# Changfei-Fu/RUMI-SLAM

Hardware: AMD Instinct MI355X
Metric: frames/sec ORB extract+match (higher is better)
Workload: dtype u8; 1 GPU; ORB extract (640x480, 8-level pyramid, 1000 features/frame) + brute-force 256-bit Hamming match of consecutive frames (BASELINE.json configs[1]+[2]); scaling=n/a (one GPU), exchange=none

## Files before the change

### rumi_slam_amd/csrc/orb_host.hip

```cpp
#include <hip/hip_runtime.h>

#include <cstdlib>

#include <algorithm>
#include <atomic>
#include <cstdio>
#include <cstring>
#include <functional>
#include <string>
#include <thread>
#include <vector>

#include "orb_device.h"
#include "orb_octree.h"
#include "rumi_common.h"

using namespace rumi;

namespace rumi {
thread_local std::string g_lastError;
void set_error(const char *fmt, const char *a, const char *b, int line) {
    char buf[512];
    snprintf(buf, sizeof buf, fmt, a, b, line);
    g_lastError = buf;
// ... 261 lines not shown
    TRY_A(dev_alloc(&h->dPyr, (size_t)h->capArena * arena));
    TRY_A(dev_alloc(&h->dBlur, (size_t)h->capArena * arena));
    TRY_A(dev_alloc(&h->dCellBuf, C * h->capCells * h->capCellCand));
    TRY_A(dev_alloc(&h->dCellCnt, C * h->capCells));
    TRY_A(dev_alloc(&h->dCand, C * h->capCand));
    TRY_A(dev_alloc(&h->dLevelStart, C * (kMaxLevels + 1)));
    TRY_A(dev_alloc(&h->dSelPacked, C * h->capSel));
    TRY_A(dev_alloc(&h->dSelMeta, C * h->capSel));
    TRY_A(dev_alloc(&h->dSelCount, C));
    TRY_A(dev_alloc(&h->dOwner, C * h->capCand));
    TRY_A(dev_alloc(&h->dSelLevel, C * h->cfg.nlevels * h->selLevelCap));
    TRY_A(dev_alloc(&h->dSelLevelCnt, C * h->cfg.nlevels));
#undef TRY_A
    h->scratchFrames = (int)scratch; h->arenaFrames = (int)arena;
    return RUMI_OK;
}

extern "C" int rumi_orb_create(const RumiOrbConfig *cfg, RumiOrb **out) {
    if (!out) return RUMI_E_INVALID;
    *out = nullptr;
    if (!cfg || cfg->nlevels < 1 || cfg->nlevels > kMaxLevels || cfg->nfeatures < 1 || cfg->max_batch < 1 ||
        cfg->max_width < 1 || cfg->max_height < 1 || !(cfg->scale_factor > 1.0f) || cfg->blur_variant < 0 || cfg->blur_variant > 1) {
        g_lastError = "invalid RumiOrbConfig";
        return RUMI_E_INVALID;
    }
    int ndev = 0;
    if (hipGetDeviceCount(&ndev) != hipSuccess || ndev == 0) {
        g_lastError = "no HIP device visible: librumi_hip has no CPU fallback";
        return RUMI_E_NO_DEVICE;
    }
    RumiOrb *h = new RumiOrb();
    h->cfg = *cfg;
    if (cfg->device >= 0) { h->device = cfg->device; }
    else if (hipGetDevice(&h->device) != hipSuccess) h->device = 0;
    if (hipSetDevice(h->device) != hipSuccess) { delete h; g_lastError = "hipSetDevice failed"; return RUMI_E_NO_DEVICE; }
    h->tab = make_tables(cfg->nfeatures, cfg->scale_factor, cfg->nlevels);
    h->hostThreads = cfg->host_threads > 0 ? cfg->host_threads
                                           : (int)std::min<unsigned>(16u, std::max(1u, std::thread::hardware_concurrency()));
    std::vector<LevelGeom> g;
    int cells, cand, cellCand;
    if (!make_geometry(h->tab, cfg->max_width, cfg->max_height, g, &h->capArena, &cells, &cand, &cellCand)) {
        delete h;
        g_lastError = "max_width x max_height too small for the FAST cell grid at some level";
        return RUMI_E_INVALID;
    }
    int coefN = 0;
    for (int l = 1; l < cfg->nlevels; l++) coefN += 3 * (g[l].w + g[l].h);
    h->capCells = cells + cells / 8 + 16;
    h->capCellCand = cellCand + cellCand / 2 + 16;
    int candSum = 0;
    for (int l = 0; l < cfg->nlevels; l++) candSum += std::min(g[l].candCap, 65535);
    h->capCand = candSum + 64;
    h->capCoef = coefN + 64 * cfg->nlevels;
    h->capRowTab = 0;
    for (int l = 1; l < cfg->nlevels; l++) h->capRowTab += g[l].h + 8;
    h->capSel = cfg->nfeatures + 4 * cfg->nlevels + 64;
    int maxN = 0;
    for (int l = 0; l < cfg->nlevels; l++) maxN = std::max(maxN, h->tab.featuresPerLevel[l]);
    h->selLevelCap = maxN + 4 * 16 + 8;
    const size_t B = (size_t)cfg->max_batch, C = (size_t)scratch_frames(cfg->max_batch);
    int rc = RUMI_OK;
#define TRY_ALLOC(x) if ((rc = (x)) != RUMI_OK) { rumi_orb_destroy(h); return rc; }
    TRY_ALLOC(dev_alloc(&h->dP, 1));
    TRY_ALLOC(dev_alloc(&h->dCoef, (size_t)h->capCoef));
    TRY_ALLOC(dev_alloc(&h->dRowTab, (size_t)std::max(h->capRowTab, 1)));
    TRY_ALLOC(dev_alloc(&h->dIn, (size_t)((cfg->max_width + 3) & ~3) * cfg->max_height));
    TRY_ALLOC(alloc_frame_arenas(h, C, B));
    TRY_ALLOC(dev_alloc(&h->dOut1, (size_t)16 + (size_t)h->capSel * 60));
    if (hipHostMalloc((void **)&h->hIn, (size_t)((cfg->max_width + 3) & ~3) * cfg->max_height, hipHostMallocDefault) != hipSuccess ||
        hipHostMalloc((void **)&h->hOut1, (size_t)16 + (size_t)h->capSel * 60, hipHostMallocDefault) != hipSuccess) {
        rumi_orb_destroy(h); g_lastError = "pinned staging"; return RUMI_E_NO_DEVICE;
    }
    TRY_ALLOC(dev_alloc(&h->dErr, 1));
    TRY_ALLOC(pin_alloc(&h->hErr, 1));
    if (hipHostGetDevicePointer((void **)&h->dhOut1, h->hOut1, 0) != hipSuccess || hipHostGetDevicePointer((void **)&h->dhErr, h->hErr, 0) != hipSuccess) {
        (void)hipGetLastError();
        h->dhOut1 = nullptr; h->dhErr = nullptr;
    }
#undef TRY_ALLOC
    for (auto &e : h->ev)
        if (hipEventCreate(&e) != hipSuccess) { rumi_orb_destroy(h); g_lastError = "hipEventCreate"; return RUMI_E_NO_DEVICE; }
    auto make_slot = [h](int p) {
        RumiOrb::Lane &L = h->slot[p];
        return hipStreamCreateWithFlags(&L.s, hipStreamNonBlocking) == hipSuccess && hipStreamCreateWithFlags(&L.bs, hipStreamNonBlocking) == hipSuccess &&
               hipEventCreateWithFlags(&L.fork, hipEventDisableTiming) == hipSuccess && hipEventCreateWithFlags(&L.join, hipEventDisableTiming) == hipSuccess &&
               hipEventCreateWithFlags(&h->slotJoin[p], hipEventDisableTiming) == hipSuccess;
    };
    bool slotsOk = true;
    for (int p = 1; p < RumiOrb::kMaxParts && slotsOk; ++p) slotsOk = make_slot(p);
    if (!slotsOk || !make_slot(0)) { rumi_orb_destroy(h); g_lastError = "slot stream"; return RUMI_E_NO_DEVICE; }
    if (hipEventCreateWithFlags(&h->evPartFork, hipEventDisableTiming) != hipSuccess ||
        hipStreamCreateWithFlags(&h->sideStream, hipStreamNonBlocking) != hipSuccess ||
        hipEventCreateWithFlags(&h->evFork, hipEventDisableTiming) != hipSuccess ||
        hipEventCreateWithFlags(&h->evJoin, hipEventDisableTiming) != hipSuccess || hipEventCreate(&h->evB0) != hipSuccess ||
        hipEventCreate(&h->evB1) != hipSuccess) { rumi_orb_destroy(h); g_lastError = "side stream"; return RUMI_E_NO_DEVICE; }
    *out = h;
    return RUMI_OK;
}

extern "C" int rumi_orb_set_profiling(RumiOrb *h, int32_t on) {
    if (!h) return RUMI_E_INVALID;
    h->profiling = on != 0;
    return RUMI_OK;
}
extern "C" int rumi_orb_set_resident_queue(RumiOrb *h, int32_t on) {
    if (!h) return RUMI_E_INVALID;
    if (h->pending) { const int rc = rumi_orb_sync(h); if (rc != RUMI_OK) return rc; }
    if (on) {
        const int slots = on == 1 ? 4 : std::min(std::max(on, 2), (int)RumiOrb::kMaxParts);
        h->residentSlots = slots;
        const int need = (slots * std::min(kResidentSub, h->cfg.max_batch) + 23) / 24 * 24;
        if (h->scratchFrames < need || h->arenaFrames < need) {
            HIP_TRY(hipSetDevice(h->device));
            HIP_TRY(hipDeviceSynchronize());
            const size_t oldS = (size_t)h->scratchFrames, oldA = (size_t)h->arenaFrames;
            int rc = alloc_frame_arenas(h, std::max(oldS, (size_t)need), std::max(oldA, (size_t)need));
            if (rc != RUMI_OK) {
                h->residentQueue = false;
                (void)alloc_frame_arenas(h, oldS, oldA);
                g_lastError = "resident queue: device arenas";
                return rc;
            }
            h->lastFrames = 0; h->tapValid = false;
        }
    }
    h->residentQueue = on != 0;
    return RUMI_OK;
}
extern "C" int rumi_orb_wait_event(RumiOrb *h, void *hip_event) {
    if (!h) return RUMI_E_INVALID;
    h->userReady = (hipEvent_t)hip_event;
    return RUMI_OK;
}
extern "C" int rumi_orb_stage_ms(RumiOrb *h, float ms[8]) {
    if (!h || !ms) return RUMI_E_INVALID;
    for (int i = 0; i < 8; i++) ms[i] = h->stageMs[i];
    return RUMI_OK;
}

extern "C" int rumi_orb_sync(RumiOrb *h) {
    if (!h) return RUMI_E_INVALID;
    if (!h->pending) return RUMI_OK;
    HIP_TRY(hipSetDevice(h->device));
    HIP_TRY(hipStreamSynchronize(h->pendingStream));
    h->pending = false;
    const int err = *h->hErr;
    if (err & 16) { g_lastError = "FAST candidate capacity exceeded (more than 65535 in one level)"; return RUMI_E_CAPACITY; }
    if (err & 1) { g_lastError = "aspect ratio gives 0 or more than 16 quadtree roots"; return RUMI_E_INVALID; }
    if (err & 2) { g_lastError = "quadtree node pool exhausted"; return RUMI_E_INVALID; }
    if (err & (4 | 8)) { g_lastError = "more key-points than the handle's selection capacity"; return RUMI_E_CAPACITY; }
    return RUMI_OK;
}

extern "C" int rumi_orb_extract_batch_device(RumiOrb *h, const void *d_imgs, int32_t nframes, int32_t w, int32_t hgt,
                                             int32_t stride, int64_t frame_stride, int32_t lap0, int32_t lap1,
                                             void *d_kp, void *d_desc, void *d_counts, int32_t cap, void *hip_stream) {
    const int rc = rumi_orb_extract_batch_device_async(h, d_imgs, nframes, w, hgt, stride, frame_stride, lap0, lap1, d_kp, d_desc, d_counts, cap, hip_stream);
    if (rc != RUMI_OK) { if (h && h->pending) (void)rumi_orb_sync(h); return rc; }
    return rumi_orb_sync(h);
}

struct OutLayout { void *kp; long long kpStride; void *desc; long long descStride; void *counts; long long countsStride; };

static int extract_async_impl(RumiOrb *h, const void *d_imgs, int32_t nframes, int32_t w, int32_t hgt, int32_t stride, int64_t frame_stride,
                              int32_t lap0, int32_t lap1, const OutLayout &out, int32_t cap, void *hip_stream) {
    void *d_kp = out.kp, *d_desc = out.desc, *d_counts = out.counts;
    if (!h || !d_imgs || !d_kp || !d_desc || !d_counts || nframes < 1 || cap < 1 || stride < w) {
        g_lastError = "rumi_orb_extract_batch_device: bad argument";
        return RUMI_E_INVALID;
    }
    if (w <= 0 || hgt <= 0) return RUMI_E_EMPTY;
    if (nframes > h->cfg.max_batch) { g_lastError = "nframes > max_batch"; return RUMI_E_CAPACITY; }
    if (h->scratchFrames <= 0 || h->arenaFrames <= 0) { g_lastError = "the handle has no device arenas (an earlier rumi_orb_set_resident_queue failed to allocate them)"; return RUMI_E_CAPACITY; }
    HIP_TRY(hipSetDevice(h->device));
    int rc;
    if (h->pending && (h->gw != w || h->gh != hgt) && (rc = rumi_orb_sync(h)) != RUMI_OK) return rc;
    rc = set_geometry(h, w, hgt);
    if (rc != RUMI_OK) return rc;
    hipStream_t st = (hipStream_t)hip_stream;
    if (h->pending && (st != h->pendingStream || h->profiling)) { rc = rumi_orb_sync(h); if (rc != RUMI_OK) return rc; }
    const DevParams &P = h->hP;
    bool stagedL0 = false;
    if ((reinterpret_cast<uintptr_t>(d_imgs) & 3) || (stride & 3) || (frame_stride & 3)) {
        stagedL0 = true;
        const int wp = (w + 3) & ~3;
        if (!h->dL0) HIP_TRY(hipMalloc((void **)&h->dL0, (size_t)((h->cfg.max_width + 3) & ~3) * h->cfg.max_height * h->cfg.max_batch));
        for (int f = 0; f < nframes; f++)
            HIP_TRY(hipMemcpy2DAsync(h->dL0 + (size_t)f * wp * hgt, wp, (const uint8_t *)d_imgs + (long long)f * frame_stride, stride, w, hgt,
                                     hipMemcpyDeviceToDevice, st));
        d_imgs = h->dL0; stride = wp; frame_stride = (int64_t)wp * hgt;
    }
    ImgSrc src{(const uint8_t *)d_imgs, frame_stride, stride, h->dPyr, h->dBlur};
    const bool prof = h->profiling;
    float acc[8] = {0};
    h->tapValid = false;

    static const bool serial = std::getenv("RUMI_SERIAL") != nullptr;
    const int parts = (!prof && !serial) ? std::min(4, std::max(nframes / 32, 1)) : 1;
    bool clearInKernel = !h->pending && parts == 1 && !(h->residentQueue && !prof && !serial && !h->feed) && P.nlevels > 1;
    if (!h->pending && !clearInKernel) HIP_TRY(hipMemsetAsync(h->dErr, 0, sizeof(int32_t), st));
    if (h->userReady && !(h->residentQueue && !prof && !serial && !h->feed)) { HIP_TRY(hipStreamWaitEvent(st, h->userReady, 0)); h->userReady = nullptr; }
    const bool resident = h->residentQueue && !prof && !serial && !h->feed;
    using Lane = RumiOrb::Lane;
    auto lane_of = [&](int slot) -> Lane {
        if (slot || resident) return h->slot[slot];
        return {st, serial || prof ? st : h->sideStream, h->evFork, h->evJoin};
    };
    const bool fuseBlur = !prof && !serial && nframes < 16 && fast_blur_fusable(P);
    const bool tilePyramid = !prof && !serial && nframes <= 4 && h->nPyrTiles > 0;
    auto stage_a = [&](const ImgSrc &ps, int n, const Lane &L) -> int {
        hipStream_t s = L.s;
        if (prof) HIP_TRY(hipEventRecord(h->ev[0], s));
        if (tilePyramid) {
            launch_pyramid_tiles(h->dP, ps, h->dCoef, h->dRowTab, h->dPyrTiles, h->nPyrTiles, h->pyrBuf, h->pyrTab, n, s, clearInKernel ? h->dErr : nullptr);
            clearInKernel = false;
        } else
        for (int l = 1; l < P.nlevels; l++) {
            launch_resize(h->dP, P, ps, h->dCoef, h->dRowTab, l, n, s, clearInKernel ? h->dErr : nullptr);
            clearInKernel = false;
        }
        if (prof) HIP_TRY(hipEventRecord(h->ev[1], s));
        if (fuseBlur) return RUMI_OK;
        HIP_TRY(hipEventRecord(L.fork, s));
        HIP_TRY(hipStreamWaitEvent(L.bs, L.fork, 0));
        if (prof) HIP_TRY(hipEventRecord(h->evB0, L.bs));
        launch_blur(h->dP, P, ps, n, h->cfg.blur_variant, L.bs);
        if (prof) HIP_TRY(hipEventRecord(h->evB1, L.bs));
        HIP_TRY(hipEventRecord(L.join, L.bs));
        HIP_TRY(hipGetLastError());
        return RUMI_OK;
    };
    if (h->hostImagePending) {
        h->hostImagePending = false;
        HIP_TRY(hipMemcpyAsync(h->dIn, h->hIn, (size_t)stride * hgt, hipMemcpyHostToDevice, st));
    }
    if (parts == 1 && !resident) {
        if (h->feed && (rc = h->feed(nframes, st)) != RUMI_OK) return rc;
        if ((rc = stage_a(src, nframes, lane_of(0))) != RUMI_OK) return rc;
    }

    auto run_part = [&](int frame0, int n, int scr0, const Lane &L, bool timed, bool withStageA, int arena0) -> int {
        hipStream_t s = L.s;
        ImgSrc ps = src;
        ps.l0 = src.l0 + (long long)frame0 * frame_stride;
        ps.pyr = src.pyr + (long long)(arena0 >= 0 ? arena0 : frame0) * P.arenaStride;
        ps.blur = src.blur + (long long)(arena0 >= 0 ? arena0 : frame0) * P.arenaStride;
        if (withStageA) { const int ra = stage_a(ps, n, L); if (ra != RUMI_OK) return ra; }
        uint32_t *cellBuf = h->dCellBuf + (size_t)scr0 * P.totalCells * P.maxCellCand;
        int32_t *cellCnt = h->dCellCnt + (size_t)scr0 * P.totalCells;
        uint32_t *candp = h->dCand + (size_t)scr0 * P.totalCand;
        int32_t *lvStart = h->dLevelStart + (size_t)scr0 * (kMaxLevels + 1);
        uint32_t *selLevel = h->dSelLevel + (size_t)scr0 * P.nlevels * h->selLevelCap;
        int32_t *selLevelCnt = h->dSelLevelCnt + (size_t)scr0 * P.nlevels;
        uint32_t *selPacked = h->dSelPacked + (size_t)scr0 * h->capSel, *selMeta = h->dSelMeta + (size_t)scr0 * h->capSel;
        if (timed) HIP_TRY(hipEventRecord(h->ev[3], s));
        if (fuseBlur) (void)launch_fast_blur(h->dP, P, ps, cellBuf, cellCnt, n, h->cfg.blur_variant, s);
        else launch_fast(h->dP, P, ps, cellBuf, cellCnt, n, s);
        if (timed) HIP_TRY(hipEventRecord(h->ev[4], s));
        launch_compact(h->dP, P, cellBuf, cellCnt, candp, lvStart, h->dErr, n, s);
        if (timed) HIP_TRY(hipEventRecord(h->ev[5], s));
        launch_octree(h->dP, P, candp, lvStart, h->dOwner + (size_t)scr0 * P.totalCand, selLevel, selLevelCnt, h->selLevelCap, h->dErr, n, h->octLds, s);
        const bool fuseAssemble = !timed && !serial && n <= 4 && (long long)((h->capSel + 7) / 8) * n <= 2048;
        int32_t *countsOut = (int32_t *)((uint8_t *)d_counts + (size_t)frame0 * out.countsStride);
        if (!fuseAssemble)
            launch_assemble(h->dP, selLevel, selLevelCnt, h->selLevelCap, lap0, lap1, selPacked, selMeta, h->dSelCount + scr0, h->capSel,
                            countsOut, out.countsStride, h->dErr, n, s, h->zeroCopyOut ? h->dhErr : nullptr);
        if (timed) HIP_TRY(hipEventRecord(h->ev[6], s));
        if (!fuseBlur) HIP_TRY(hipStreamWaitEvent(s, L.join, 0));
        if (fuseAssemble)
            launch_assemble_orient_desc(h->dP, ps, selLevel, selLevelCnt, h->selLevelCap, lap0, lap1, countsOut, out.countsStride, h->dErr,
                                        h->zeroCopyOut ? h->dhErr : nullptr, selPacked, selMeta, h->dSelCount + scr0, h->capSel, h->capSel,
                                        (RumiKeyPoint *)((uint8_t *)d_kp + (size_t)frame0 * out.kpStride), out.kpStride,
                                        (uint8_t *)d_desc + (size_t)frame0 * out.descStride, out.descStride, cap, n, s);
        else
        launch_orient_desc(h->dP, ps, selPacked, selMeta, h->dSelCount + scr0, h->capSel, h->capSel,
                           (RumiKeyPoint *)((uint8_t *)d_kp + (size_t)frame0 * out.kpStride), out.kpStride,
                           (uint8_t *)d_desc + (size_t)frame0 * out.descStride, out.descStride, cap, n, s);
        if (timed) HIP_TRY(hipEventRecord(h->ev[7], s));
        const RumiOrb::Mirror &mr = h->mirror;
        if (mr.host) HIP_TRY(hipMemcpyAsync(mr.host + (size_t)frame0 * mr.row, mr.dev + (size_t)frame0 * mr.row, (size_t)n * mr.row, hipMemcpyDeviceToHost, s));
        return RUMI_OK;
    };
    if (resident) {
        constexpr int kMaxSlots = RumiOrb::kMaxParts;
        const int kSlots = h->residentSlots;
        const int slotFrames = h->scratchFrames / kSlots;
        const int cap64 = std::min(kResidentSub, slotFrames);
        const int nsub = (nframes + cap64 - 1) / cap64, sub = (nframes + nsub - 1) / nsub;
        const bool fork = !h->pending || !h->lastResident || stagedL0;
        if (fork) HIP_TRY(hipEventRecord(h->evPartFork, st));
        bool touched[kMaxSlots] = {false, false, false, false, false, false, false, false};
        for (int j = 0, base = 0; base < nframes; j++, base += sub) {
            const int n = std::min(sub, nframes - base), slot = (h->rot + j) % kSlots;
            const Lane L = lane_of(slot);
            if (fork && !touched[slot]) HIP_TRY(hipStreamWaitEvent(L.s, h->evPartFork, 0));
            if (h->userReady && !touched[slot]) HIP_TRY(hipStreamWaitEvent(L.s, h->userReady, 0));
            touched[slot] = true;
            rc = run_part(base, n, slot * slotFrames, L, false, true, slot * slotFrames);
            if (rc != RUMI_OK) return rc;
            h->lastChunkBase = base; h->lastChunkFrames = n; h->lastChunkSlot = slot * slotFrames;
        }
        h->rot = (h->rot + nsub) % kSlots;
        h->userReady = nullptr;
        for (int p = 0; p < kSlots; p++)
            if (touched[p]) {
// ... 322 lines not shown
```

### rumi_slam_amd/csrc/orb_kernels.hip

```cpp
#include <hip/hip_runtime.h>

#include "orb_device.h"
#include "orb_math.h"

namespace rumi {

struct PatternF { float v[256 * 4]; };
constexpr PatternF make_pattern_f() {
    constexpr int8_t src[256 * 4] = {
#include "orb_pattern.inc"
    };
    PatternF p{};
    for (int i = 0; i < 256 * 4; i++) p.v[i] = (float)src[i];
    return p;
}
__constant__ PatternF c_patternF = make_pattern_f();

__device__ __forceinline__ unsigned xcd_swizzle(unsigned lin, unsigned total) {
    const unsigned q = total >> 3, r = total & 7, xcd = lin & 7;
    return (xcd < r ? xcd * (q + 1) : r * (q + 1) + (xcd - r) * q) + (lin >> 3);
}

struct __attribute__((packed)) U32 { uint32_t v; };
struct __attribute__((packed)) U64 { uint64_t v; };
// ... 499 lines not shown
    if (r0 < rps && c < g.nd) {
        const uint8_t *src = g.img + r0 * g.pitch + 4 * c;
        uint8_t *dst = tile + r0 * TP + 4 * c;
        const int nb = (g.rows + rps - 1) / rps, lastRow = g.rows - rps;
        uint32_t v[kStageDepth];
#pragma unroll
        for (int j = 0; j < kStageDepth; j++)
            if (j < nb) v[j] = reinterpret_cast<const U32 *>(src + (long long)min(j * rps, lastRow) * g.pitch)->v;
#pragma unroll
        for (int j = 0; j < kStageDepth; j++)
            if (j < nb) *reinterpret_cast<uint32_t *>(dst + min(j * rps, lastRow) * TP) = v[j];
        for (int j = kStageDepth; j < nb; j++)
            *reinterpret_cast<uint32_t *>(dst + min(j * rps, lastRow) * TP) = reinterpret_cast<const U32 *>(src + (long long)min(j * rps, lastRow) * g.pitch)->v;
    }
}

template <int TPC>
__device__ __forceinline__ void fast_cell_process(const DevParams *__restrict__ P, const FastLds &F, const FastCell &g, uint8_t *tile, uint8_t *sc,
                                                  uint32_t *__restrict__ cellBuf, int32_t *__restrict__ cellCnt, int lane) {
    const int TP = TPC ? TPC : F.tp;
    const int dw = g.cols - 6, dh = g.rows - 6;
    const unsigned Mdw = magic_of(dw), Mtp = magic_of(TP);
    for (int idx = lane * 16; idx < (dh + 2) * TP; idx += 1024) *reinterpret_cast<uint4 *>(&sc[idx]) = make_uint4(0, 0, 0, 0);
    wave_lds_fence();
    const int npx = dw * dh;
    const int scDelta = -2 * TP - 3;
    uint16_t *cl = reinterpret_cast<uint16_t *>(sc + F.scBytes);
    uint16_t *sl = cl + kRingCap;
    int thr = max(1, P->iniTh);
    uint32_t *out = cellBuf + g.cellIdx * P->maxCellCand;
    int found;
#pragma nounroll
    for (int pass = 0;; pass++) {
        const int nScored = fast_score_cell_bytes<TPC>(tile, sc, cl, sl, TP, dw, dh, thr, lane);
        wave_lds_fence();
        const bool listed = nScored <= kScoredCap;
        const int nItems = listed ? nScored : npx;
        found = 0;
        for (int base = 0; base < nItems; base += 128) {
            int si[2];
            bool in[2];
#pragma unroll
            for (int h = 0; h < 2; h++) {
                const int k = base + 64 * h + lane;
                in[h] = k < nItems;
                if (listed) {
                    si[h] = (int)sl[in[h] ? k : 0] + scDelta;
                } else {
                    const int kk = in[h] ? k : 0, py = magic_div(kk, Mdw);
                    si[h] = mul24(py + 1, TP) + (kk - mul24(py, dw)) + 1;
                }
            }
            int v[2];
            bool isMax[2];
#pragma unroll
            for (int h = 0; h < 2; h++) {
                const uint8_t *s = &sc[si[h]];
                v[h] = s[0];
                const int n0 = s[-TP - 1], n1 = s[-TP], n2 = s[-TP + 1], n3 = s[-1], n4 = s[1], n5 = s[TP - 1], n6 = s[TP], n7 = s[TP + 1];
                isMax[h] = in[h] & (v[h] > 0) & (v[h] > n0) & (v[h] > n1) & (v[h] > n2) & (v[h] > n3) & (v[h] > n4) & (v[h] > n5) & (v[h] > n6) & (v[h] > n7);
            }
            const unsigned long long b0 = __ballot(isMax[0]), b1 = __ballot(isMax[1]);
            const int c0 = __popcll(b0);
#pragma unroll
            for (int h = 0; h < 2; h++) {
                if (isMax[h]) {
                    const unsigned long long b = h ? b1 : b0;
                    const int slot = __builtin_amdgcn_mbcnt_hi((uint32_t)(b >> 32), __builtin_amdgcn_mbcnt_lo((uint32_t)b, found + (h ? c0 : 0)));
                    const int py1 = magic_div(si[h], Mtp), px1 = si[h] - mul24(py1, TP);
                    const uint32_t x = (uint32_t)(px1 + 2 + g.ox), y = (uint32_t)(py1 + 2 + g.oy);
                    out[slot] = x | (y << 12) | ((uint32_t)v[h] << 24);
                }
            }
            found += c0 + __popcll(b1);
        }
        if (found > 0 || pass == 1) break;
        thr = max(1, P->minTh);
    }
    if (lane == 0) cellCnt[g.cellIdx] = found;
}

template <int TPC>
__device__ __forceinline__ void fast_cells_body(const DevParams *__restrict__ P, const ImgSrc &src, const FastLds &F, uint32_t *__restrict__ cellBuf,
                                                int32_t *__restrict__ cellCnt, unsigned bx, unsigned gx) {
    extern __shared__ __attribute__((aligned(16))) uint8_t fl[];
    const int lane = threadIdx.x & 63, wave = __builtin_amdgcn_readfirstlane(threadIdx.x >> 6);
    const unsigned wg = xcd_swizzle(blockIdx.y * gx + bx, gx * gridDim.y);
    const int wpg = blockDim.x >> 6;
    const int cell = (wg % gx) * wpg + wave, frame = wg / gx;
    uint8_t *tile = fl + (size_t)wave * F.perWave;
    uint8_t *sc = tile + F.tileBytes;
    const int TP = TPC ? TPC : F.tp;
    const FastCell gA = fast_cell_geom(P, src, cell, frame, cellCnt, lane);
    if (!gA.live) return;
    fast_cell_stage<TPC>(gA, tile, TP, lane);
    fast_cell_process<TPC>(P, F, gA, tile, sc, cellBuf, cellCnt, lane);
}
template <int TPC>
__global__ __launch_bounds__(256) void k_fast_cells(const DevParams *__restrict__ P, ImgSrc src, FastLds F,
                                                    uint32_t *__restrict__ cellBuf, int32_t *__restrict__ cellCnt) {
    fast_cells_body<TPC>(P, src, F, cellBuf, cellCnt, blockIdx.x, gridDim.x);
}

constexpr int kCompactThreads = 256;
__global__ __launch_bounds__(kCompactThreads) void k_compact(const DevParams *__restrict__ P, const uint32_t *__restrict__ cellBuf,
                                                 const int32_t *__restrict__ cellCnt, uint32_t *__restrict__ cand,
                                                 int32_t *__restrict__ levelStart, int32_t *__restrict__ errFlag) {
    extern __shared__ int sStart[];
    __shared__ int part[kCompactThreads];
    const int tid = threadIdx.x, frame = blockIdx.x;
    const int nc = P->totalCells;
    const int32_t *cnt = cellCnt + (long long)frame * nc;
    const int chunk = (nc + kCompactThreads - 1) / kCompactThreads;
    int sum = 0;
    for (int k = 0; k < chunk; k++) {
        const int c = tid * chunk + k;
        if (c < nc) sum += cnt[c];
    }
    const int lane = tid & 63, wave = __builtin_amdgcn_readfirstlane(tid >> 6);
    int inc = sum;
#pragma unroll
    for (int o = 1; o < 64; o <<= 1) {
        const int t = __shfl_up(inc, o);
        if (lane >= o) inc += t;
    }
    if (lane == 63) part[wave] = inc;
    __syncthreads();
    int base = 0, total = 0;
#pragma unroll
    for (int w = 0; w < kCompactThreads / 64; w++) {
        const int t = part[w];
        if (w < wave) base += t;
        total += t;
    }
    if (tid == 0) sStart[nc] = total;
    int run = base + inc - sum;
    for (int k = 0; k < chunk; k++) {
        const int c = tid * chunk + k;
        if (c < nc) { sStart[c] = run; run += cnt[c]; }
    }
    __syncthreads();
    int32_t *ls = levelStart + (long long)frame * (kMaxLevels + 1);
    if (blockIdx.y == 0 && tid <= P->nlevels) {
        const int c = tid < P->nlevels ? P->lv[tid].cellBase : nc;
        ls[tid] = sStart[c];
    }
    if (blockIdx.y == 0 && tid < P->nlevels) {
        const int c0 = P->lv[tid].cellBase, c1 = c0 + P->lv[tid].nCells;
        if (sStart[c1] - sStart[c0] > P->lv[tid].candCap) atomicOr(errFlag, 16);
    }
    uint32_t *out = cand + (long long)frame * P->totalCand;
    const int nOut = min(sStart[nc], P->totalCand);
    const uint32_t *inBase = cellBuf + (long long)frame * nc * P->maxCellCand;
    for (int j = blockIdx.y * kCompactThreads + tid; j < nOut; j += kCompactThreads * gridDim.y) {
        int lo = 0, hi = nc;
        while (hi - lo > 1) {
            const int mid = (lo + hi) >> 1;
            if (sStart[mid] <= j) lo = mid; else hi = mid;
        }
        out[j] = inBase[(long long)lo * P->maxCellCand + (j - sStart[lo])];
    }
}

constexpr int kBlurRowsSmall = 16, kBlurRowsBatch = 64;

struct BlurGrid { int base[kMaxLevels + 1]; int gx[kMaxLevels]; int bw[kMaxLevels]; };
__device__ __forceinline__ uint32_t mad_u24(uint32_t a, uint32_t b, uint32_t c) {
    uint32_t r;
    asm("v_mad_u32_u24 %0, %1, %2, %3" : "=v"(r) : "v"(a), "v"(b), "v"(c));
    return r;
}
template <int VARIANT, int kBlurRows>
__device__ __forceinline__ void blur_body(const DevParams *__restrict__ P, const ImgSrc &src, const BlurGrid &G, unsigned bxg, unsigned gxg) {
    constexpr uint32_t kT2 = VARIANT ? 49u : 48u, kT3 = VARIANT ? 55u : 56u;
    const int lane = threadIdx.x & 63, wave = __builtin_amdgcn_readfirstlane(threadIdx.x >> 6);
    const unsigned wg = xcd_swizzle(blockIdx.y * gxg + bxg, gxg * gridDim.y);
    const int frame = wg / gxg, lin = wg % gxg;
    int level = 0;
    for (int l = 1; l < P->nlevels; l++)
        if (lin >= G.base[l]) level = l;
    const DevLevel &L = P->lv[level];
    const int bx = (lin - G.base[level]) % G.gx[level], by = (lin - G.base[level]) / G.gx[level];
    const int bw = G.bw[level];
    const int xa = bx * bw + lane * 4;
    const int y0 = (by * 4 + wave) * kBlurRows;
    if (y0 >= L.h) return;
    int pitch;
    const uint8_t *img = level_base(src, P, level, frame, &pitch);
    uint8_t *out = src.blur + (long long)frame * P->arenaStride + L.off;
    const int w = L.w, h = L.h;
    const int xLast = (w - 1) & ~3;
    const int xl = min(xa, xLast);
    const bool firstBlock = bx == 0;
    const bool edgeWave = bx * bw + bw + 4 > w;
    const bool produce = lane * 4 < bw && xa < w;
    uint32_t selA = 0x03020100u, selB = 0x07060504u;
    if (edgeWave && xa + 3 >= w && xa <= xLast + 4) {
#pragma unroll
        for (int i = 0; i < 4; i++) {
            const int x = xa + i;
            if (x < w) continue;
            const int sx = 2 * (w - 1) - x, d = (xa - (sx & ~3)) >> 2;
            const uint32_t a = (d == 1 ? 4u : 0u) + (uint32_t)(sx & 3);
            const uint32_t b = d == 0 ? 4u + (uint32_t)(sx & 3) : (uint32_t)i;
            selA = (selA & ~(0xFFu << (8 * i))) | (a << (8 * i));
            selB = (selB & ~(0xFFu << (8 * i))) | (b << (8 * i));
        }
    }
    int ring[7][4];
#pragma unroll
    for (int k = 0; k < 7; k++)
#pragma unroll
        for (int i = 0; i < 4; i++) ring[k][i] = 0;
    const int yEnd = min(y0 + kBlurRows, h), rEnd = yEnd + 3;
    uint8_t *orow = out + (long long)(y0 - 6) * L.pitch + xa - L.pitch;
    const int haloOff = lane == 0 ? (firstBlock ? 0 : -4) : (lane == 63 && !edgeWave && bw == 256 ? 4 : 0);
    uint32_t Cn[7], Hn[7];
    auto fetch = [&](int r, uint32_t &C, uint32_t &H) {
        const int rc = min(r, rEnd - 1);
        const int rr = rc < 0 ? -rc : (rc >= h ? 2 * (h - 1) - rc : rc);
        const uint8_t *row = img + (long long)rr * pitch + xl;
        C = *reinterpret_cast<const uint32_t *>(row);
        H = 0;
        if (haloOff) H = *reinterpret_cast<const uint32_t *>(row + haloOff);
    };
#pragma unroll
    for (int j = 0; j < 7; j++) fetch(y0 - 3 + j, Cn[j], Hn[j]);
    uint32_t Cm[7], Hm[7];
    auto walk7 = [&](const uint32_t (&Cc)[7], const uint32_t (&Hc)[7], int r0) {
#pragma unroll
        for (int j = 0; j < 7; j++) {
            const int r = r0 + j;
            if (r >= rEnd) break;
            orow += L.pitch;
            uint32_t C = Cc[j];
            if (edgeWave) {
                const uint32_t c1 = __shfl_up(C, 1), c2 = __shfl_up(c1, 1);
                C = __builtin_amdgcn_perm(C, __builtin_amdgcn_perm(c1, c2, selA), selB);
            }
            uint32_t Lw = __shfl_up(C, 1), Rw = __shfl_down(C, 1);
            if (lane == 0) Lw = firstBlock ? __builtin_amdgcn_perm(C, C, 0x01020300u) : Hc[j];
            if (lane == 63 && !edgeWave && bw == 256) Rw = Hc[j];
            constexpr uint32_t tA = 18u | (34u << 8) | (kT2 << 16) | (kT3 << 24), tB = kT2 | (34u << 8) | (18u << 16);
            const uint32_t A0 = __builtin_amdgcn_alignbyte(C, Lw, 1), A1 = __builtin_amdgcn_alignbyte(C, Lw, 2), A2 = __builtin_amdgcn_alignbyte(C, Lw, 3);
            const uint32_t B0 = __builtin_amdgcn_alignbyte(Rw, C, 1), B1 = __builtin_amdgcn_alignbyte(Rw, C, 2), B2 = __builtin_amdgcn_alignbyte(Rw, C, 3);
            ring[j][0] = (int)__builtin_amdgcn_udot4(B0, tB, __builtin_amdgcn_udot4(A0, tA, 0u, false), false);
            ring[j][1] = (int)__builtin_amdgcn_udot4(B1, tB, __builtin_amdgcn_udot4(A1, tA, 0u, false), false);
            ring[j][2] = (int)__builtin_amdgcn_udot4(B2, tB, __builtin_amdgcn_udot4(A2, tA, 0u, false), false);
            ring[j][3] = (int)__builtin_amdgcn_udot4(Rw, tB, __builtin_amdgcn_udot4(C, tA, 0u, false), false);
            const int y = r - 3;
            if (y >= y0 && produce) {
                uint32_t o[4];
#pragma unroll
                for (int i = 0; i < 4; i++) {
                    uint32_t acc = mad_u24(kT3, (uint32_t)ring[(j + 4) % 7][i], 32768u);
                    acc = mad_u24(kT2, (uint32_t)(ring[(j + 3) % 7][i] + ring[(j + 5) % 7][i]), acc);
                    acc = mad_u24(34u, (uint32_t)(ring[(j + 2) % 7][i] + ring[(j + 6) % 7][i]), acc);
                    acc = mad_u24(18u, (uint32_t)(ring[(j + 1) % 7][i] + ring[j][i]), acc);
                    if (VARIANT) acc = min(acc, 0x00FFFFFFu);
                    o[i] = acc;
                }
                const uint32_t p01 = __builtin_amdgcn_perm(o[1], o[0], 0x0c0c0602u), p23 = __builtin_amdgcn_perm(o[3], o[2], 0x06020c0cu);
                *reinterpret_cast<uint32_t *>(orow) = p01 | p23;
            }
        }
    };
    for (int r0 = y0 - 3; r0 < rEnd; r0 += 7) {
#pragma unroll
        for (int j = 0; j < 7; j++) Cm[j] = Cn[j], Hm[j] = Hn[j];
        if (r0 + 7 < rEnd) {
#pragma unroll
            for (int j = 0; j < 7; j++) fetch(r0 + 7 + j, Cn[j], Hn[j]);
        }
        walk7(Cm, Hm, r0);
    }
}
template <int VARIANT, int kBlurRows>
__global__ __launch_bounds__(256) void k_blur(const DevParams *__restrict__ P, ImgSrc src, BlurGrid G) {
    blur_body<VARIANT, kBlurRows>(P, src, G, blockIdx.x, gridDim.x);
}
template <int TPC, int VARIANT>
__global__ __launch_bounds__(256) void k_fast_blur(const DevParams *__restrict__ P, ImgSrc src, FastLds F, uint32_t *__restrict__ cellBuf,
                                                   int32_t *__restrict__ cellCnt, BlurGrid G, unsigned gxFast) {
    if (blockIdx.x < gxFast) fast_cells_body<TPC>(P, src, F, cellBuf, cellCnt, blockIdx.x, gxFast);
    else blur_body<VARIANT, kBlurRowsSmall>(P, src, G, blockIdx.x - gxFast, gridDim.x - gxFast);
}

__device__ __forceinline__ int half_wave_sum(int v) {
    v += __builtin_amdgcn_update_dpp(0, v, 0x111, 0xF, 0xF, false);
    v += __builtin_amdgcn_update_dpp(0, v, 0x112, 0xF, 0xF, false);
    v += __builtin_amdgcn_update_dpp(0, v, 0x114, 0xF, 0xF, false);
    v += __builtin_amdgcn_update_dpp(0, v, 0x118, 0xF, 0xF, false);
    v += __builtin_amdgcn_update_dpp(0, v, 0x142, 0xA, 0xF, false);
    const int lo = __builtin_amdgcn_readlane(v, 31), hi = __builtin_amdgcn_readlane(v, 63);
    return (threadIdx.x & 32) ? hi : lo;
}
__device__ __forceinline__ int wave_sum(int v) {
#pragma unroll
    for (int o = 32; o > 0; o >>= 1) v += __shfl_xor(v, o);
    return v;
}

constexpr int kDiscP = 48, kPatchP = 48;
constexpr int kKpPerWg = 8;

struct AssembleArgs {
    const uint32_t *selLevel; const int32_t *selLevelCnt; int selLevelCap, lap0, lap1;
    int32_t *counts; long long countsStride; int32_t *errFlag, *errMirror;
    uint32_t *selPackedOut, *selMetaOut; int32_t *selCountOut;
};
template <int kKpGroups, bool kAssemble>
__global__ __launch_bounds__(256, 7) void k_orient_desc(const DevParams *__restrict__ P, ImgSrc src,
                                                     const uint32_t *__restrict__ selPacked,
                                                     const uint32_t *__restrict__ selMeta,
                                                     const int32_t *__restrict__ selCount, int selCap,
                                                     RumiKeyPoint *__restrict__ kpOut, long long kpStride, uint8_t *__restrict__ descOut,
                                                     long long descStride, int outCap, AssembleArgs A) {
    static_assert(kDiscP == kPatchP, "the disc and the patch share their rows");
    __shared__ __attribute__((aligned(16))) uint8_t sWin[kKpPerWg][37 * kPatchP];
    __shared__ __attribute__((aligned(16))) float sPat[256 * 4];
    __shared__ int4 sLv[kMaxLevels];
    __shared__ float2 sLvF[kMaxLevels];
    reinterpret_cast<float4 *>(sPat)[threadIdx.x] = reinterpret_cast<const float4 *>(c_patternF.v)[threadIdx.x];
    if (threadIdx.x < (unsigned)P->nlevels) {
        const DevLevel &Lv = P->lv[threadIdx.x];
        sLv[threadIdx.x] = threadIdx.x == 0 ? make_int4(0, src.l0Pitch, (int)Lv.off, Lv.pitch) : make_int4((int)Lv.off, Lv.pitch, (int)Lv.off, Lv.pitch);
        sLvF[threadIdx.x] = make_float2(Lv.scale, Lv.patchSize);
    }
    const int lane = threadIdx.x & 31, hw = threadIdx.x >> 5;
    const unsigned wg = xcd_swizzle(blockIdx.y * gridDim.x + blockIdx.x, gridDim.x * gridDim.y);
    const int kb = (wg % gridDim.x) * (kKpPerWg * kKpGroups) + hw, frame = wg / gridDim.x;
    int cnt;
    __shared__ uint32_t sOwnPk[kAssemble ? kKpPerWg * kKpGroups : 1], sOwnMt[kAssemble ? kKpPerWg * kKpGroups : 1];
    if constexpr (!kAssemble) {
        cnt = selCount[frame];
        __syncthreads();
    } else {
        __shared__ int sLvStart[kMaxLevels + 1], sRed[2], sOwnF[kKpPerWg * kKpGroups];
        const int nl = P->nlevels, tid = threadIdx.x;
        if (tid == 0) {
            int run = 0;
            for (int l = 0; l < nl; l++) { sLvStart[l] = run; run += A.selLevelCnt[(long long)frame * nl + l]; }
            sLvStart[nl] = run; sRed[0] = 0; sRed[1] = 0;
        }
        __syncthreads();
        const int total = sLvStart[nl], kbase = (wg % gridDim.x) * (kKpPerWg * kKpGroups);
        const bool first = wg % gridDim.x == 0, over = total > selCap;
        int32_t *counts = reinterpret_cast<int32_t *>(reinterpret_cast<uint8_t *>(A.counts) + frame * A.countsStride);
        if (over) {
            if (first && tid == 0) { A.selCountOut[frame] = 0; counts[0] = total; counts[1] = 0; const int old = atomicOr(A.errFlag, 8); if (A.errMirror) *A.errMirror = old | 8; }
            return;
        }
        cnt = total;
        auto key_at = [&](int k, int *levelOut) -> uint32_t {
            int level = 0;
            while (k >= sLvStart[level + 1]) level++;
            *levelOut = level;
            return A.selLevel[((long long)frame * nl + level) * A.selLevelCap + (k - sLvStart[level])];
        };
        auto lapped = [&](uint32_t pk, int level) -> bool {
            float x = (float)((int)(pk & 0xFFF) + kBorder);
            if (level != 0) x = x * P->lv[level].scale;
            return x >= (float)A.lap0 && x <= (float)A.lap1;
        };
        int before = 0, all = 0;
        for (int k = tid; k < total; k += 256) {
            int level;
            const uint32_t pk = key_at(k, &level);
// ... 169 lines not shown
        stage_patch(liveC, S);
        if (g + 1 < kKpGroups) fetch_patch(pkN, mtN, liveN, S);
        if (liveC) describe(pkC, mtC, angle);
        OD_STAMP(3);
        pkC = pkN; mtC = mtN; liveC = liveN;
        pkN = pkNN; mtN = mtNN; liveN = liveNN;
    }
#ifdef RUMI_OD_STAMP
    if (threadIdx.x == 0 && (blockIdx.x % 8) == 0 && blockIdx.y == 0) printf("od wg %d: loop-head %lld stage(wait loads) %lld issue-next %lld | IC_Angle %lld trig %lld rBRIEF %lld store %lld\n", (int)blockIdx.x, st[0], st[1], st[2], st[4], st[5], st[6], st[3]);
#endif
}

void launch_resize(const DevParams *dP, const DevParams &hP, ImgSrc src, const int16_t *coef, const RowTap *rowTab, int level, int nframes,
                   hipStream_t st, int32_t *clearWord) {
    const int rows = hP.lv[level].h >= 200 ? 8 : 4;
    dim3 g((hP.lv[level].w + 255) / 256, (hP.lv[level].h + 4 * rows - 1) / (4 * rows), nframes);
    if (rows == 8) hipLaunchKernelGGL(k_resize<8>, g, dim3(256), 0, st, dP, src, coef, rowTab, level, clearWord);
    else hipLaunchKernelGGL(k_resize<4>, g, dim3(256), 0, st, dP, src, coef, rowTab, level, clearWord);
}
void launch_pyramid_tiles(const DevParams *dP, ImgSrc src, const int16_t *coef, const RowTap *rowTab, const PyrTile *tiles, int ntiles, int bufBytes,
                          int tabEntries, int nframes, hipStream_t st, int32_t *clearWord) {
    hipLaunchKernelGGL(k_pyramid_tiles, dim3(ntiles, nframes), dim3(256), (size_t)2 * bufBytes + (size_t)tabEntries * 8, st, dP, src, coef, rowTab, tiles, bufBytes, clearWord);
}
static FastLds fast_lds_of(const DevParams &hP) {
    int wMax = 0, hMax = 0;
    for (int l = 0; l < hP.nlevels; l++) { wMax = std::max(wMax, hP.lv[l].wCell); hMax = std::max(hMax, hP.lv[l].hCell); }
    FastLds F;
    F.tp = 4 * (((wMax + 3) >> 2) + 2);
    F.sp = F.tp;
    F.tileBytes = (hMax + 6) * F.tp;
    F.scBytes = ((hMax + 2) * F.sp + 15) & ~15;
    F.maxIters = (wMax * hMax + 63) / 64 + 1;
    F.tileBytes = (F.tileBytes + 15) & ~15;
    F.perWave = (F.tileBytes + F.scBytes + std::max(kRingCap * 2, F.maxIters * 8) + kScoredCap * 2 + 15) & ~15;
    return F;
}
void launch_fast(const DevParams *dP, const DevParams &hP, ImgSrc src, uint32_t *cellBuf, int32_t *cellCnt, int nframes,
                 hipStream_t st) {
    const FastLds F = fast_lds_of(hP);
    const int wpg = 4;
    const dim3 grid((hP.totalCells + wpg - 1) / wpg, nframes);
    const size_t lds = (size_t)wpg * F.perWave;
#define RUMI_FAST_CASE(T)                                                                                      \
    if (F.tp == T) {                                                                                           \
        hipLaunchKernelGGL((k_fast_cells<T>), grid, dim3(64 * wpg), lds, st, dP, src, F, cellBuf, cellCnt);    \
        return;                                                                                                \
    }
    RUMI_FAST_CASE(48) RUMI_FAST_CASE(44) RUMI_FAST_CASE(52) RUMI_FAST_CASE(56)
#undef RUMI_FAST_CASE
    hipLaunchKernelGGL((k_fast_cells<0>), grid, dim3(64 * wpg), lds, st, dP, src, F, cellBuf, cellCnt);
}
static int compactSlices(int nframes) { return nframes < 32 ? 32 : 8; }
void launch_compact(const DevParams *dP, const DevParams &hP, const uint32_t *cellBuf, const int32_t *cellCnt,
                    uint32_t *cand, int32_t *levelStart, int32_t *errFlag, int nframes, hipStream_t st) {
    hipLaunchKernelGGL(k_compact, dim3(nframes, compactSlices(nframes)), dim3(kCompactThreads), (hP.totalCells + 1) * sizeof(int), st, dP, cellBuf, cellCnt,
                       cand, levelStart, errFlag);
}
static int blur_strip_width(int w) {
    for (int bw : {256, 240, 224, 208}) {
        const int r = w % bw;
        const bool partialInFirstLanes = r >= 1 && r <= 8;
        const bool lane63Halo = bw == 256 && (r >= 253 || r <= 3);
        if (!partialInFirstLanes && !lane63Halo) return bw;
    }
    return 192;
}
static BlurGrid blur_grid_of(const DevParams &hP, int rows, int *total) {
    BlurGrid G{};
    int run = 0;
    for (int l = 0; l < hP.nlevels; l++) {
        G.bw[l] = blur_strip_width(hP.lv[l].w);
        G.gx[l] = (hP.lv[l].w + G.bw[l] - 1) / G.bw[l];
        G.base[l] = run;
        run += G.gx[l] * ((hP.lv[l].h + 4 * rows - 1) / (4 * rows));
    }
    G.base[hP.nlevels] = run;
    *total = run;
    return G;
}
bool fast_blur_fusable(const DevParams &hP) { return fast_lds_of(hP).tp == 48; }
bool launch_fast_blur(const DevParams *dP, const DevParams &hP, ImgSrc src, uint32_t *cellBuf, int32_t *cellCnt, int nframes, int variant, hipStream_t st) {
    const FastLds F = fast_lds_of(hP);
    if (F.tp != 48) return false;
    int run = 0;
    const BlurGrid G = blur_grid_of(hP, kBlurRowsSmall, &run);
    const int wpg = 4;
    const unsigned gxFast = (unsigned)((hP.totalCells + wpg - 1) / wpg);
    const dim3 grid(gxFast + (unsigned)run, nframes);
    const size_t lds = (size_t)wpg * F.perWave;
    if (variant) hipLaunchKernelGGL((k_fast_blur<48, 1>), grid, dim3(256), lds, st, dP, src, F, cellBuf, cellCnt, G, gxFast);
    else hipLaunchKernelGGL((k_fast_blur<48, 0>), grid, dim3(256), lds, st, dP, src, F, cellBuf, cellCnt, G, gxFast);
    return true;
}
void launch_blur(const DevParams *dP, const DevParams &hP, ImgSrc src, int nframes, int variant, hipStream_t st) {
    const bool small = nframes < 16;
    const int rows = small ? kBlurRowsSmall : kBlurRowsBatch;
    int run = 0;
    const BlurGrid G = blur_grid_of(hP, rows, &run);
    if (small) {
        if (variant) hipLaunchKernelGGL((k_blur<1, kBlurRowsSmall>), dim3(run, nframes), dim3(256), 0, st, dP, src, G);
        else hipLaunchKernelGGL((k_blur<0, kBlurRowsSmall>), dim3(run, nframes), dim3(256), 0, st, dP, src, G);
    } else {
        if (variant) hipLaunchKernelGGL((k_blur<1, kBlurRowsBatch>), dim3(run, nframes), dim3(256), 0, st, dP, src, G);
        else hipLaunchKernelGGL((k_blur<0, kBlurRowsBatch>), dim3(run, nframes), dim3(256), 0, st, dP, src, G);
    }
}
void launch_orient_desc(const DevParams *dP, ImgSrc src, const uint32_t *selPacked, const uint32_t *selMeta,
                        const int32_t *selCount, int selCap, int maxSel, RumiKeyPoint *kpOut, long long kpStride, uint8_t *descOut,
                        long long descStride, int outCap, int nframes, hipStream_t st) {
    if (maxSel <= 0) return;
    const int wg1 = (maxSel + kKpPerWg - 1) / kKpPerWg;
    const AssembleArgs none{};
    if ((long long)wg1 * nframes <= 2048)
        hipLaunchKernelGGL((k_orient_desc<1, false>), dim3(wg1, nframes), dim3(256), 0, st, dP, src, selPacked, selMeta, selCount, selCap, kpOut, kpStride, descOut,
                           descStride, outCap, none);
    else
        hipLaunchKernelGGL((k_orient_desc<2, false>), dim3((wg1 + 1) / 2, nframes), dim3(256), 0, st, dP, src, selPacked, selMeta, selCount, selCap, kpOut, kpStride,
                           descOut, descStride, outCap, none);
}
void launch_assemble_orient_desc(const DevParams *dP, ImgSrc src, const uint32_t *selLevel, const int32_t *selLevelCnt, int selLevelCap, int lap0, int lap1,
                                 int32_t *counts, long long countsStride, int32_t *errFlag, int32_t *errMirror, uint32_t *selPacked, uint32_t *selMeta,
                                 int32_t *selCount, int selCap, int maxSel, RumiKeyPoint *kpOut,
                                 long long kpStride, uint8_t *descOut, long long descStride, int outCap, int nframes, hipStream_t st) {
    if (maxSel <= 0) return;
    const int wg1 = (maxSel + kKpPerWg - 1) / kKpPerWg;
    const AssembleArgs A{selLevel, selLevelCnt, selLevelCap, lap0, lap1, counts, countsStride, errFlag, nframes == 1 ? errMirror : nullptr, selPacked, selMeta, selCount};
    hipLaunchKernelGGL((k_orient_desc<1, true>), dim3(wg1, nframes), dim3(256), 0, st, dP, src, (const uint32_t *)nullptr, (const uint32_t *)nullptr,
                       (const int32_t *)nullptr, selCap, kpOut, kpStride, descOut, descStride, outCap, A);
}

}
```

Measured before the change: 287,100 frames/s.

## Extend fused FAST+blur kernel to batched frames and interleave blur blocks

Removes the nframes<16 restriction so the fused FAST-cells plus blur kernel also runs for large batches, with a batch-sized blur row count. Inside the fused kernel, blur and FAST work groups are interleaved evenly across the XCD-swizzled block index instead of being split into two contiguous ranges, and the swizzle is applied over the combined grid. Side blur streams are now created lazily only when the separate blur path is actually needed. This drops the fork/join to a side stream and a separate blur launch for batched runs, at the cost of mixing two kernels with different register and LDS needs in one launch.

```diff
diff --git a/rumi_slam_amd/csrc/orb_host.hip b/rumi_slam_amd/csrc/orb_host.hip
--- a/rumi_slam_amd/csrc/orb_host.hip
+++ b/rumi_slam_amd/csrc/orb_host.hip
@@ -367,15 +367,14 @@
         if (hipEventCreate(&e) != hipSuccess) { rumi_orb_destroy(h); g_lastError = "hipEventCreate"; return RUMI_E_NO_DEVICE; }
     auto make_slot = [h](int p) {
         RumiOrb::Lane &L = h->slot[p];
-        return hipStreamCreateWithFlags(&L.s, hipStreamNonBlocking) == hipSuccess && hipStreamCreateWithFlags(&L.bs, hipStreamNonBlocking) == hipSuccess &&
+        return hipStreamCreateWithFlags(&L.s, hipStreamNonBlocking) == hipSuccess &&
                hipEventCreateWithFlags(&L.fork, hipEventDisableTiming) == hipSuccess && hipEventCreateWithFlags(&L.join, hipEventDisableTiming) == hipSuccess &&
                hipEventCreateWithFlags(&h->slotJoin[p], hipEventDisableTiming) == hipSuccess;
     };
     bool slotsOk = true;
-    for (int p = 1; p < RumiOrb::kMaxParts && slotsOk; ++p) slotsOk = make_slot(p);
-    if (!slotsOk || !make_slot(0)) { rumi_orb_destroy(h); g_lastError = "slot stream"; return RUMI_E_NO_DEVICE; }
+    for (int p = 0; p < RumiOrb::kMaxParts && slotsOk; ++p) slotsOk = make_slot(p);
+    if (!slotsOk) { rumi_orb_destroy(h); g_lastError = "slot stream"; return RUMI_E_NO_DEVICE; }
     if (hipEventCreateWithFlags(&h->evPartFork, hipEventDisableTiming) != hipSuccess ||
-        hipStreamCreateWithFlags(&h->sideStream, hipStreamNonBlocking) != hipSuccess ||
         hipEventCreateWithFlags(&h->evFork, hipEventDisableTiming) != hipSuccess ||
         hipEventCreateWithFlags(&h->evJoin, hipEventDisableTiming) != hipSuccess || hipEventCreate(&h->evB0) != hipSuccess ||
         hipEventCreate(&h->evB1) != hipSuccess) { rumi_orb_destroy(h); g_lastError = "side stream"; return RUMI_E_NO_DEVICE; }
@@ -486,12 +485,15 @@
     if (!h->pending && !clearInKernel) HIP_TRY(hipMemsetAsync(h->dErr, 0, sizeof(int32_t), st));
     if (h->userReady && !(h->residentQueue && !prof && !serial && !h->feed)) { HIP_TRY(hipStreamWaitEvent(st, h->userReady, 0)); h->userReady = nullptr; }
     const bool resident = h->residentQueue && !prof && !serial && !h->feed;
+    const bool fuseBlur = !prof && !serial && fast_blur_fusable(P);
     using Lane = RumiOrb::Lane;
     auto lane_of = [&](int slot) -> Lane {
-        if (slot || resident) return h->slot[slot];
+        const bool own = slot || resident;
+        hipStream_t *bs = own ? &h->slot[slot].bs : &h->sideStream;
+        if (!fuseBlur && !prof && !serial && !*bs && hipStreamCreateWithFlags(bs, hipStreamNonBlocking) != hipSuccess) *bs = nullptr;
+        if (own) return h->slot[slot];
         return {st, serial || prof ? st : h->sideStream, h->evFork, h->evJoin};
     };
-    const bool fuseBlur = !prof && !serial && nframes < 16 && fast_blur_fusable(P);
     const bool tilePyramid = !prof && !serial && nframes <= 4 && h->nPyrTiles > 0;
     auto stage_a = [&](const ImgSrc &ps, int n, const Lane &L) -> int {
         hipStream_t s = L.s;
@@ -506,6 +508,7 @@
         }
         if (prof) HIP_TRY(hipEventRecord(h->ev[1], s));
         if (fuseBlur) return RUMI_OK;
+        if (!L.bs) { g_lastError = "side stream"; return RUMI_E_NO_DEVICE; }
         HIP_TRY(hipEventRecord(L.fork, s));
         HIP_TRY(hipStreamWaitEvent(L.bs, L.fork, 0));
         if (prof) HIP_TRY(hipEventRecord(h->evB0, L.bs));
diff --git a/rumi_slam_amd/csrc/orb_kernels.hip b/rumi_slam_amd/csrc/orb_kernels.hip
--- a/rumi_slam_amd/csrc/orb_kernels.hip
+++ b/rumi_slam_amd/csrc/orb_kernels.hip
@@ -605,12 +605,11 @@
 
 template <int TPC>
 __device__ __forceinline__ void fast_cells_body(const DevParams *__restrict__ P, const ImgSrc &src, const FastLds &F, uint32_t *__restrict__ cellBuf,
-                                                int32_t *__restrict__ cellCnt, unsigned bx, unsigned gx) {
+                                                int32_t *__restrict__ cellCnt, unsigned lin, int frame) {
     extern __shared__ __attribute__((aligned(16))) uint8_t fl[];
     const int lane = threadIdx.x & 63, wave = __builtin_amdgcn_readfirstlane(threadIdx.x >> 6);
-    const unsigned wg = xcd_swizzle(blockIdx.y * gx + bx, gx * gridDim.y);
     const int wpg = blockDim.x >> 6;
-    const int cell = (wg % gx) * wpg + wave, frame = wg / gx;
+    const int cell = lin * wpg + wave;
     uint8_t *tile = fl + (size_t)wave * F.perWave;
     uint8_t *sc = tile + F.tileBytes;
     const int TP = TPC ? TPC : F.tp;
@@ -622,7 +621,8 @@
 template <int TPC>
 __global__ __launch_bounds__(256) void k_fast_cells(const DevParams *__restrict__ P, ImgSrc src, FastLds F,
                                                     uint32_t *__restrict__ cellBuf, int32_t *__restrict__ cellCnt) {
-    fast_cells_body<TPC>(P, src, F, cellBuf, cellCnt, blockIdx.x, gridDim.x);
+    const unsigned wg = xcd_swizzle(blockIdx.y * gridDim.x + blockIdx.x, gridDim.x * gridDim.y);
+    fast_cells_body<TPC>(P, src, F, cellBuf, cellCnt, wg % gridDim.x, wg / gridDim.x);
 }
 
 constexpr int kCompactThreads = 256;
@@ -686,6 +686,7 @@
 }
 
 constexpr int kBlurRowsSmall = 16, kBlurRowsBatch = 64;
+constexpr int kBlurSmallFrames = 16;
 
 struct BlurGrid { int base[kMaxLevels + 1]; int gx[kMaxLevels]; int bw[kMaxLevels]; };
 __device__ __forceinline__ uint32_t mad_u24(uint32_t a, uint32_t b, uint32_t c) {
@@ -694,11 +695,9 @@
     return r;
 }
 template <int VARIANT, int kBlurRows>
-__device__ __forceinline__ void blur_body(const DevParams *__restrict__ P, const ImgSrc &src, const BlurGrid &G, unsigned bxg, unsigned gxg) {
+__device__ __forceinline__ void blur_body(const DevParams *__restrict__ P, const ImgSrc &src, const BlurGrid &G, int lin, int frame) {
     constexpr uint32_t kT2 = VARIANT ? 49u : 48u, kT3 = VARIANT ? 55u : 56u;
     const int lane = threadIdx.x & 63, wave = __builtin_amdgcn_readfirstlane(threadIdx.x >> 6);
-    const unsigned wg = xcd_swizzle(blockIdx.y * gxg + bxg, gxg * gridDim.y);
-    const int frame = wg / gxg, lin = wg % gxg;
     int level = 0;
     for (int l = 1; l < P->nlevels; l++)
         if (lin >= G.base[l]) level = l;
@@ -800,13 +799,18 @@
 }
 template <int VARIANT, int kBlurRows>
 __global__ __launch_bounds__(256) void k_blur(const DevParams *__restrict__ P, ImgSrc src, BlurGrid G) {
-    blur_body<VARIANT, kBlurRows>(P, src, G, blockIdx.x, gridDim.x);
-}
-template <int TPC, int VARIANT>
+    const unsigned wg = xcd_swizzle(blockIdx.y * gridDim.x + blockIdx.x, gridDim.x * gridDim.y);
+    blur_body<VARIANT, kBlurRows>(P, src, G, wg % gridDim.x, wg / gridDim.x);
+}
+template <int TPC, int VARIANT, int kBlurRows>
 __global__ __launch_bounds__(256) void k_fast_blur(const DevParams *__restrict__ P, ImgSrc src, FastLds F, uint32_t *__restrict__ cellBuf,
-                                                   int32_t *__restrict__ cellCnt, BlurGrid G, unsigned gxFast) {
-    if (blockIdx.x < gxFast) fast_cells_body<TPC>(P, src, F, cellBuf, cellCnt, blockIdx.x, gxFast);
-    else blur_body<VARIANT, kBlurRowsSmall>(P, src, G, blockIdx.x - gxFast, gridDim.x - gxFast);
+                                                   int32_t *__restrict__ cellCnt, BlurGrid G, unsigned gxFast, unsigned gxBlur) {
+    const unsigned gx = gxFast + gxBlur;
+    const unsigned wg = xcd_swizzle(blockIdx.y * gx + blockIdx.x, gx * gridDim.y);
+    const unsigned frame = wg / gx, pos = wg % gx;
+    const unsigned b0 = pos * gxBlur / gx, b1 = (pos + 1) * gxBlur / gx;
+    if (b1 > b0) blur_body<VARIANT, kBlurRows>(P, src, G, b0, frame);
+    else fast_cells_body<TPC>(P, src, F, cellBuf, cellCnt, pos - b0, frame);
 }
 
 __device__ __forceinline__ int half_wave_sum(int v) {
@@ -1142,18 +1146,21 @@
 bool launch_fast_blur(const DevParams *dP, const DevParams &hP, ImgSrc src, uint32_t *cellBuf, int32_t *cellCnt, int nframes, int variant, hipStream_t st) {
     const FastLds F = fast_lds_of(hP);
     if (F.tp != 48) return false;
+    const bool small = nframes < kBlurSmallFrames;
     int run = 0;
-    const BlurGrid G = blur_grid_of(hP, kBlurRowsSmall, &run);
+    const BlurGrid G = blur_grid_of(hP, small ? kBlurRowsSmall : kBlurRowsBatch, &run);
     const int wpg = 4;
     const unsigned gxFast = (unsigned)((hP.totalCells + wpg - 1) / wpg);
     const dim3 grid(gxFast + (unsigned)run, nframes);
     const size_t lds = (size_t)wpg * F.perWave;
-    if (variant) hipLaunchKernelGGL((k_fast_blur<48, 1>), grid, dim3(256), lds, st, dP, src, F, cellBuf, cellCnt, G, gxFast);
-    else hipLaunchKernelGGL((k_fast_blur<48, 0>), grid, dim3(256), lds, st, dP, src, F, cellBuf, cellCnt, G, gxFast);
+#define RUMI_FAST_BLUR(V, R) hipLaunchKernelGGL((k_fast_blur<48, V, R>), grid, dim3(256), lds, st, dP, src, F, cellBuf, cellCnt, G, gxFast, (unsigned)run)
+    if (small) { if (variant) RUMI_FAST_BLUR(1, kBlurRowsSmall); else RUMI_FAST_BLUR(0, kBlurRowsSmall); }
+    else { if (variant) RUMI_FAST_BLUR(1, kBlurRowsBatch); else RUMI_FAST_BLUR(0, kBlurRowsBatch); }
+#undef RUMI_FAST_BLUR
     return true;
 }
 void launch_blur(const DevParams *dP, const DevParams &hP, ImgSrc src, int nframes, int variant, hipStream_t st) {
-    const bool small = nframes < 16;
+    const bool small = nframes < kBlurSmallFrames;
     const int rows = small ? kBlurRowsSmall : kBlurRowsBatch;
     int run = 0;
     const BlurGrid G = blur_grid_of(hP, rows, &run);
```

Measured after the change: 279,300 frames/s. -2.7%, worse.
